# feifeibear/long-context-attention

Hardware: AMD Instinct MI355X
Metric: attention TFLOP/s (algorithmic, causal fwd+bwd) + iter ms of LongContextAttention at seqlen 64K, ulysses x ring (higher is better)
Workload: dtype bf16

## Files before the change

long-context-attention_amd/csrc/usp_flash_bwd64.hip:

```cpp
#ifdef USP_B64_TIMING
#define USP_TIMING
#endif
#include "usp_bwd_params.hpp"
#include "usp_host.hpp"
#include "usp_mfma64.hpp"

namespace usp {

#ifndef USP_B64_STATW
#define USP_B64_STATW 0
#endif
constexpr int kB64_STATW = USP_B64_STATW;
#ifndef USP_B64_DMA_PH
#define USP_B64_DMA_PH 0
#endif
constexpr int kB64_DMA_PH = USP_B64_DMA_PH;
#ifndef USP_B64_E0
#define USP_B64_E0 20
#endif
constexpr int kB64_E0 = USP_B64_E0;
#ifndef USP_B64_E1
#define USP_B64_E1 54
#endif
constexpr int kB64_E1 = USP_B64_E1;


template <int DT, bool CAUSAL>
__global__ __launch_bounds__(256, 1) void flash_bwd_dkdv64_kernel(const BwdParams ) {
  using E = Elem<DT>;
  using M = M64<DT>;
  constexpr int D = 128, OWN = 128;
  constexpr int ROWB = D * 2;
  constexpr int TILEB = kTile * ROWB;
  constexpr int STATB = 2 * kTile * 4;
  constexpr int BUFB = 2 * TILEB + STATB;
  constexpr int NBUF = 3;
  constexpr int PSLOT = 8192;
  constexpr int POFF = NBUF * BUFB;
  constexpr int NKT = D / 16, NDJ = D / 32;

  extern __shared__ __attribute__((aligned(16))) char smem_raw[];
  USP_LDS char* smem = lds_block_at_zero(smem_raw);

  const int tid = threadIdx.x;
  const int lane = tid & 63;
  const int wave = __builtin_amdgcn_readfirstlane(tid >> 6);
  const int role = wave >> 1;
  const int slice = wave & 1;
  const int l31 = lane & 31;
  const int hi = lane >> 5;
  typedef const __attribute__((address_space(4))) BwdParams* KArgs;
  KArgs p = (KArgs)__builtin_amdgcn_kernarg_segment_ptr();
  asm volatile("" : "+s"(p));

  const int dma_row = lane >> 4;
  const int dma_c8 = ((lane & 15) ^ ((lane >> 4) << 2)) * 16;
  const int q_voff = dma_row * (int)p->q_ss * 2 + dma_c8, do_voff = dma_row * (int)p->do_ss * 2 + dma_c8;
  const int rd_base = l31 * ROWB + ((hi ^ tile_swz<D>(l31)) * 16);
  int tr_addr[NDJ][2];
  {
    const int i = lane & 15, grp = (lane >> 4) & 1;
#pragma unroll
    for (int dj = 0; dj < NDJ; ++dj)
#pragma unroll
      for (int e = 0; e < 2; ++e) tr_addr[dj][e] = tr_read_offset<D>(i, grp, hi, dj, e);
  }
  USP_LDS char* pex = smem + POFF + slice * 2 * PSLOT + lane * 16;

  const ItemWalk walk(p->n_items);
  for (int pass = 0;; ++pass) {
  int w = walk.at(pass);
  if (w < 0) break;
  asm volatile("" : "+s"(p));
  USP_TM(const uint64_t tm_item = __builtin_amdgcn_s_memtime();)
  w = walk.dealt(w, p->nblk);
  const int blk = w % p->nblk;
  int rest = w / p->nblk;
  int g = 0, cut = 0;
  if (p->qsplit > 1) { cut = rest % p->qsplit; rest /= p->qsplit; }
  if (p->ngrp > 1) { g = rest % p->ngrp; rest /= p->ngrp; }
  const int hkv = rest % p->Hkv, b = rest / p->Hkv;
  const int gsub = p->gsub;
  const int h0 = hkv * p->G + g * gsub;
  const int own0 = blk * OWN;
  const int off = p->causal_off;
  const int ow = own0 + slice * 64;

  u32x4 rf[2][NKT];
  {
    const char* pr[2];
#pragma unroll
    for (int kb = 0; kb < 2; ++kb) {
      const int orow = ow + 32 * kb + l31;
      const int orow_c = orow < p->Sk ? orow : p->Sk - 1;
      pr[kb] = (role == 0 ? p->k + 2 * (b * p->k_sb + (int64_t)orow_c * p->k_ss + hkv * p->k_sh)
                          : p->v + 2 * (b * p->v_sb + (int64_t)orow_c * p->v_ss + hkv * p->v_sh)) + 16 * hi;
    }
    load_resident16(rf[0], rf[1], pr[0], pr[1]);
  }

  {
#pragma unroll
    for (int kb = 0; kb < 2; ++kb)
#pragma unroll
      for (int t = 0; t < NKT; ++t) pin_agpr4(rf[kb][t]);
  }
  const float c2 = p->scale_log2;
  const float neg_inv_scale = -__builtin_amdgcn_rcpf(p->scale);

  int t_end = (p->Sq + kTile - 1) / kTile;
  int t_begin = usp_first_row_tile(own0, CAUSAL, off, t_end, kTile);
  if (p->qsplit > 1) {
    const int per = (t_end - t_begin + p->qsplit - 1) / p->qsplit;
    t_begin = usp_run_begin(t_begin, t_end, per, cut);
    t_end = usp_run_end(t_begin, t_end, per);
  }
  const int n_iter = t_end - t_begin;

  const int64_t tb1 = (int64_t)kTile * p->q_ss * 2, tb2 = (int64_t)kTile * p->do_ss * 2;
  int q_step = 4 * (int)p->q_ss * 2 - 1024, do_step = 4 * (int)p->do_ss * 2 - 1024;
  const int q_rowb = (int)p->q_ss * 2, do_rowb = (int)p->do_ss * 2;
  const int gq = role == 0 ? slice : 2 + slice, gd = 2 * slice;
  int lds_q = gq * 4096, lds_d = TILEB + gd * 4096;
  const char *q_cur = nullptr, *do_cur = nullptr;
  int rows_q = 0, rows_d = 0;

  const float *lse_h = nullptr, *dl_h = nullptr;
  int st_row = 0;
  float st_lse = 0.f, st_delta = 0.f;
  bool st_in = false;
  const bool stat_wave = wave == kB64_STATW;
  auto pf_head = [&](int h) {
    q_cur = p->q + 2 * (b * p->q_sb + h * p->q_sh) + t_begin * tb1 + (int64_t)gq * 16 * q_rowb;
    do_cur = p->dout + 2 * (b * p->do_sb + h * p->do_sh) + t_begin * tb2 + (int64_t)gd * 16 * do_rowb;
    rows_q = p->Sq - t_begin * kTile - 16 * gq;
    rows_d = p->Sq - t_begin * kTile - 16 * gd;
    lse_h = p->lse + b * p->lse_sb + h * p->lse_sh;
    dl_h = p->delta + b * p->dl_sb + h * p->dl_sh;
    st_row = t_begin * kTile;
  };
  u32x4 q_rs, do_rs;
  int dma_buf = 0;
  auto dma_open = [&](int buf) {
    q_rs = make_rsrc_rows(q_cur, rows_q, 16, q_rowb, 2 * D);
    do_rs = make_rsrc_rows(do_cur, rows_d, 32, do_rowb, 2 * D);
    dma_buf = buf;
    q_cur += tb1;
    do_cur += tb2;
    rows_q -= kTile;
    rows_d -= kTile;
  };
  auto stats_fetch = [&]() {
    if (stat_wave) {
      const int r = st_row + lane;
      st_in = r < p->Sq;
      const int rc = st_in ? r : p->Sq - 1;
      const float* pl = lse_h + rc;
      const float* pd = dl_h + rc;
      asm volatile("global_load_dword %0, %2, off\n\tglobal_load_dword %1, %3, off" : "=&v"(st_lse), "=&v"(st_delta) : "v"(pl), "v"(pd) : "memory");
    }
    st_row += kTile;
  };
  auto dma_piece = [&](int n) {
    asm volatile("" : "+s"(lds_q), "+s"(lds_d), "+s"(q_step), "+s"(do_step));
    const int i = n & 3;
    if (n < 4) lds_dma16_asm(q_rs, lds_q + dma_buf * BUFB, q_voff ^ (16 * i), i * q_step, i);
    else if (n < 8) lds_dma16_asm(do_rs, lds_d + dma_buf * BUFB, do_voff ^ (16 * i), i * do_step, i);
    else lds_dma16_asm(do_rs, lds_d + 4096 + dma_buf * BUFB, do_voff ^ (16 * i), 4096 + 4 * do_step + i * do_step, i);
  };
  auto stats_store = [&](int buf) {
    if (stat_wave) {
      asm volatile("" : "+v"(st_lse), "+v"(st_delta));
      const float l2 = (st_in && st_lse != USP_NEG_INF) ? st_lse * neg_inv_scale : -__builtin_inff();
      *(USP_LDS float*)(smem + buf * BUFB + 2 * TILEB + 4 * lane) = l2;
      *(USP_LDS float*)(smem + buf * BUFB + 2 * TILEB + 4 * kTile + 4 * lane) = st_in ? -st_delta : 0.f;
    }
  };

  f32x16 acc[2][NDJ];
#pragma unroll
  for (int kb = 0; kb < 2; ++kb)
#pragma unroll
    for (int dj = 0; dj < NDJ; ++dj) zero_pin_agpr(acc[kb][dj]);

  const int n_mask = usp_masked_row_tiles(ow, CAUSAL, off, t_begin, n_iter, kTile);
  int tile_cur = t_begin, buf_a = 0, buf_b = NBUF - 1;
USP_TM(
  uint64_t tm_body = 0, tm_drain = 0, tm_bar = 0, tm_last = __builtin_amdgcn_s_memtime();
  const uint64_t tm_loop = tm_last;
)
  u32x4 fc0[NKT];
  f32x16 cst0;
#pragma unroll
  for (int kt = 0; kt < NKT; ++kt) fc0[kt] = u32x4{0u, 0u, 0u, 0u};
#pragma unroll
  for (int r = 0; r < 16; ++r) cst0[r] = 0.f;
  auto step = [&](auto role_c, auto mask_c, int it, bool work) __attribute__((always_inline)) {
    constexpr int ROLE = decltype(role_c)::value;
    constexpr bool MASK = decltype(mask_c)::value;
    constexpr int E0 = kB64_E0, E1 = kB64_E1;
    static_assert(E0 >= 16 && E1 <= 56 && E1 > E0, "");
    const int buf_n = buf_a + 1 == NBUF ? 0 : buf_a + 1;
    stats_fetch();
    int krn = rd_base + buf_a * BUFB + TILEB;
    asm volatile("" : "+v"(krn));
    auto next_c = [&](int kt) { fc0[kt] = *(USP_LDS const u32x4*)(smem + (krn ^ (32 * kt))); };
    auto next_s = [&](int j) {
      const f32x4 t = *(USP_LDS const f32x4*)(smem + buf_a * BUFB + 2 * TILEB + 4 * kTile + 16 * hi + 32 * j);
#pragma unroll
      for (int e = 0; e < 4; ++e) cst0[4 * j + e] = t[e];
    };
    if (work) {
#pragma unroll
      for (int kb = 0; kb < 2; ++kb)
#pragma unroll
        for (int t = 0; t < NKT; ++t) pin_agpr4(rf[kb][t]);
      const int my_it = it - ROLE;
      const int buf = ROLE == 0 ? buf_a : buf_b;
      const int s0 = (ROLE == 0 ? tile_cur : tile_cur - 1) * kTile;
      USP_LDS const char* x1 = smem + buf * BUFB;
      USP_LDS const char* x2 = x1 + TILEB;
      USP_LDS const char* xg = ROLE == 0 ? x2 : x1;
      USP_LDS const char* stat = x1 + 2 * TILEB + (ROLE == 0 ? 0 : 4 * kTile) + 16 * hi;
      USP_LDS char* pslot = pex + (my_it & 1) * PSLOT;
      f32x16 sc[2][2];
      u32x4 pk[2][2][2];
      u32x4 pin[2][2][2];
      f32x16 cst[2];
      int kr = rd_base + buf * BUFB + (ROLE == 0 ? 0 : TILEB);
      asm volatile("" : "+v"(kr));
      auto load_stats = [&](int h) {
        if (ROLE == 1 && h == 0) { cst[0] = cst0; return; }
#pragma unroll
        for (int j = 0; j < 4; ++j) {
          const f32x4 t = *(USP_LDS const f32x4*)(stat + 128 * h + 32 * j);
#pragma unroll
          for (int e = 0; e < 4; ++e) cst[h][4 * j + e] = t[e];
        }
      };
      auto elem = [&](int h, int n) {
        const int k2 = n >> 4, kb = (n >> 3) & 1, r = 8 * k2 + (n & 7);
        float val;
        if (ROLE == 0) {
          val = fast_exp2(sc[h][kb][r] * c2);
        } else {
          const uint32_t wd = pin[h][kb][k2][(r & 7) >> 1];
          val = ((r & 1) ? E::hi(wd) : E::lo(wd)) * sc[h][kb][r];
        }
        sc[h][kb][r] = val;
      };
      auto elem_pack = [&](int h, int n) {
        const int k2 = n >> 4, kb = (n >> 3) & 1, r = 8 * k2 + (n & 7);
        if (r & 1) pk[h][kb][k2][(r & 7) >> 1] = E::pack2(sc[h][kb][r - 1], sc[h][kb][r]);
        if (ROLE == 0 && (r & 7) == 7)
          *(USP_LDS u32x4*)(pslot + ((2 * h + kb) * 2 + k2) * 1024) = pk[h][kb][k2];
      };
      constexpr int LAG = ROLE == 0 ? 2 : 0;
      auto elem_slot = [&](int sl) {
        if (sl < E0 || sl >= E1) return;
#pragma unroll
        for (int n = (sl - E0) * 64 / (E1 - E0); n < (sl - E0 + 1) * 64 / (E1 - E0); ++n) {
          elem(n >> 5, n & 31);
          if (n >= LAG) elem_pack((n - LAG) >> 5, (n - LAG) & 31);
        }
        if (sl == E1 - 1) {
#pragma unroll
          for (int n = 64 - LAG; n < 64; ++n) elem_pack(n >> 5, n & 31);
        }
      };
      auto apply_mask = [&](int h) {
#pragma unroll
        for (int kb = 0; kb < 2; ++kb) {
          const int d = ow + 32 * kb + l31 - off - s0 - 4 * hi - 32 * h;
#pragma unroll
          for (int r = 0; r < 16; ++r)
            if (d > (r & 3) + 8 * (r >> 2)) sc[h][kb][r] = USP_NEG_INF;
        }
      };
      u32x4 fc[2][NKT];
      u32x4 xa[2][2 * NDJ];
      auto rd_c = [&](int h, int kt) { fc[h][kt] = *(USP_LDS const u32x4*)(smem + h * 32 * ROWB + (kr ^ (32 * kt))); };
      auto rd_g = [&](int h, int f) {
        USP_LDS const char* xb = xg + (2 * h + f / NDJ) * 16 * ROWB;
        const u32x2 a0 = lds_read_tr16(xb + tr_addr[f % NDJ][0]);
        const u32x2 a1 = lds_read_tr16(xb + tr_addr[f % NDJ][1]);
        xa[h][f] = u32x4{a0[0], a0[1], a1[0], a1[1]};
      };
      auto chain_init = [&](int h) {
        load_stats(h);
        if (ROLE == 1) {
#pragma unroll
          for (int kb = 0; kb < 2; ++kb)
#pragma unroll
            for (int k2 = 0; k2 < 2; ++k2) pin[h][kb][k2] = *(USP_LDS const u32x4*)(pslot + ((2 * h + kb) * 2 + k2) * 1024);
        }
      };
      auto chain_phase = [&](int h) {
#pragma unroll
        for (int sl = 0; sl < 16; ++sl) {
          const int kt = sl >> 1, kb = sl & 1;
          if (kt == 0) M::template s_first_c<MASK>(sc[h][kb], fc[h][kt], rf[kb][kt], cst[h]);
          else M::template s_next<MASK>(sc[h][kb], fc[h][kt], rf[kb][kt]);
          if (h == kB64_DMA_PH && sl == 0) {
            __builtin_amdgcn_sched_barrier(0);
            dma_open(buf_n);
          }
          if (sl < NKT) { if (h == 0) rd_c(1, sl); else rd_g(0, sl); }
          if (h == 0 && sl == 8) chain_init(1);
          elem_slot(16 * h + sl);
          if (h == kB64_DMA_PH) {
            if (ROLE == 0 && (sl & 3) == 1) dma_piece(sl >> 2);
            if (ROLE == 1 && sl >= 1 && sl <= 12) dma_piece(sl - 1);
          }
          __builtin_amdgcn_sched_barrier(0);
        }
      };
      auto grad_phase = [&](int h) {
#pragma unroll
        for (int i = 0; i < 16; ++i) {
          const int f = i >> 1, kb = i & 1;
          M::template o_acc<MASK>(acc[kb][f % NDJ], xa[h][f], pk[h][kb][f / NDJ]);
          if (h == 0 && i < 2 * NDJ) rd_g(1, i);
          if (ROLE == 1 && h == 1 && i >= 8) next_c(i - 8);
          if (ROLE == 1 && h == 1 && i >= 4 && i < 8) next_s(i - 4);
          elem_slot(32 + 16 * h + i);
          __builtin_amdgcn_sched_barrier(0);
        }
      };
      chain_init(0);
      if (ROLE == 1) {
#pragma unroll
        for (int kt = 0; kt < NKT; ++kt) fc[0][kt] = fc0[kt];
      } else {
#pragma unroll
        for (int kt = 0; kt < NKT; ++kt) rd_c(0, kt);
      }
      __builtin_amdgcn_sched_barrier(0);
      chain_phase(0);
      if (MASK) { mfma_settle(sc[0]); apply_mask(0); }
      __builtin_amdgcn_s_waitcnt(0xc07f);
      chain_phase(1);
      if (MASK) { mfma_settle(sc[1]); apply_mask(1); }
      __builtin_amdgcn_s_waitcnt(0xc07f);
      grad_phase(0);
      __builtin_amdgcn_s_waitcnt(0xc07f);
      grad_phase(1);
    } else {
      dma_open(buf_n);
#pragma unroll
      for (int n = 0; n < (ROLE == 0 ? 4 : 12); ++n) dma_piece(n);
    }
    if (ROLE == 1 && !work) {
#pragma unroll
      for (int kt = 0; kt < NKT; ++kt) next_c(kt);
#pragma unroll
      for (int j = 0; j < 4; ++j) next_s(j);
    }
    buf_b = buf_a;
    buf_a = buf_n;
    if (ROLE == 0 || it > 0) ++tile_cur;
    USP_TM(const uint64_t tm0 = __builtin_amdgcn_s_memtime();)
    dma_drain();
    USP_TM(const uint64_t tm1 = __builtin_amdgcn_s_memtime();)
    stats_store(buf_n);
    __syncthreads();
    USP_TM(const uint64_t tm2 = __builtin_amdgcn_s_memtime();
           tm_body += tm0 - tm_last; tm_drain += tm1 - tm0; tm_bar += tm2 - tm1; tm_last = tm2;)
  };
  const std::integral_constant<int, 0> rA;
  const std::integral_constant<int, 1> rB;
  const std::integral_constant<bool, false> plain;
  const std::integral_constant<bool, true> masked;
  auto open_head = [&](int h) {
    pf_head(h);
    stats_fetch();
    dma_open(0);
#pragma unroll
    for (int n = 0; n < 4; ++n) dma_piece(n);
    if (role == 1) {
#pragma unroll
      for (int n = 4; n < 12; ++n) dma_piece(n);
    }
    dma_drain();
    stats_store(0);
    __syncthreads();
    tile_cur = t_begin; buf_a = 0; buf_b = NBUF - 1;
  };
  if (role == 0) {
    for (int hh = 0; hh < gsub; ++hh) {
      open_head(h0 + hh);
      int it = 0;
      __builtin_amdgcn_s_waitcnt(0x0f70);
      for (; it < n_mask; ++it) step(rA, masked, it, true);
      __builtin_amdgcn_s_waitcnt(0x0f70);
      for (; it < n_iter; ++it) step(rA, plain, it, true);
      mfma_settle(acc);
      step(rA, plain, n_iter, false);
    }
  } else {
    for (int hh = 0; hh < gsub; ++hh) {
      open_head(h0 + hh);
      step(rB, plain, 0, false);
      __builtin_amdgcn_s_waitcnt(0x0f70);
      for (int it = 1; it <= n_iter; ++it) step(rB, plain, it, true);
      mfma_settle(acc);
    }
  }

  mfma_settle(acc);
USP_TM(
  const uint64_t tm_epi = __builtin_amdgcn_s_memtime();
  if (pass == 0 && lane == 0 && (blockIdx.x % 61) == 0)
    printf("TM wg %3d wave %d blk %2d n_iter %3d : body %8llu drain %7llu barrier %7llu  (per iteration %5llu / %4llu / %4llu)\n",
           (int)blockIdx.x, wave, blk, n_iter, (unsigned long long)tm_body, (unsigned long long)tm_drain,
           (unsigned long long)tm_bar, (unsigned long long)(tm_body / (n_iter + 1)), (unsigned long long)(tm_drain / (n_iter + 1)),
           (unsigned long long)(tm_bar / (n_iter + 1)));
)
  asm volatile("" : "+s"(p));
  const bool wide = !p->split && (p->wide16 & (role == 0 ? 4 : 2)) != 0;
#pragma unroll
  for (int kb = 0; kb < 2; ++kb) {
    const int orow = ow + 32 * kb + l31;
    if (wide) {
      const int orow_c = orow < p->Sk ? orow : 0;
      char* row16 = role == 0 ? p->dv16 + 2 * (b * p->dv16_sb + (int64_t)orow_c * p->dv16_ss + hkv * p->dv16_sh)
                              : p->dk16 + 2 * (b * p->dk16_sb + (int64_t)orow_c * p->dk16_ss + hkv * p->dk16_sh);
      store_row16_wide<E, NDJ>(row16, acc[kb], role == 0 ? 1.f : p->scale, hi, orow < p->Sk);
    } else if (orow < p->Sk) {
      float* o32;
      char* o16 = nullptr;
      int accf;
      const float mul = role == 0 ? 1.f : p->scale;
      if (p->split) {
        const int64_t wo = (((int64_t)(g * p->qsplit + cut) * p->ws_rows + (int64_t)b * p->Sk + orow) * p->Hkv + hkv) * D;
        o32 = (role == 0 ? p->ws_dv : p->ws_dk) + wo; accf = 0;
      } else if (role == 0) {
        o32 = p->dv + b * p->dv_sb + (int64_t)orow * p->dv_ss + hkv * p->dv_sh; accf = p->accum_dv;
        if (p->dv16) o16 = p->dv16 + 2 * (b * p->dv16_sb + (int64_t)orow * p->dv16_ss + hkv * p->dv16_sh);
      } else {
        o32 = p->dk + b * p->dk_sb + (int64_t)orow * p->dk_ss + hkv * p->dk_sh; accf = p->accum_dk;
        if (p->dk16) o16 = p->dk16 + 2 * (b * p->dk16_sb + (int64_t)orow * p->dk16_ss + hkv * p->dk16_sh);
      }
      store_row32_acc<E, NDJ>(o32, o16, acc[kb], mul, hi, accf);
    }
  }
USP_TM(
  if (pass < 3 && lane == 0 && (blockIdx.x % 61) == 0)
    printf("TI wg %3d pass %d wave %d blk %2d n_iter %3d n_mask %d : prologue %6llu loops %8llu epilogue %6llu\n", (int)blockIdx.x, pass,
           wave, blk, n_iter, n_mask, (unsigned long long)(tm_loop - tm_item), (unsigned long long)(tm_epi - tm_loop),
           (unsigned long long)(__builtin_amdgcn_s_memtime() - tm_epi));
)
  }
}

bool dkdv64_serves(const BwdParams& p_in) {
  if (p_in.seq_q || p_in.seq_k || p_in.sched || p_in.win_on) return false;
  return dma_rows_ok(p_in.q_ss, true) && dma_rows_ok(p_in.do_ss, true);
}

bool launch_dkdv64(const BwdParams& p_in, int dtype, bool causal, hipStream_t st, int* rc) {
  if (!dkdv64_serves(p_in)) return false;
  BwdParams p = p_in;
  p.wide16 = ((p.dk16 && !p.accum_dk && tensor_aligned(p.dk16, p.dk16_sb, p.dk16_ss, p.dk16_sh, 16, 8)) ? 2 : 0) |
             ((p.dv16 && !p.accum_dv && tensor_aligned(p.dv16, p.dv16_sb, p.dv16_ss, p.dv16_sh, 16, 8)) ? 4 : 0);
  p.nblk = (p.Sk + 127) / 128;
  p.n_items = p.B * p.Hkv * p.nblk * p.ngrp * p.qsplit;
  const int grid = persistent_grid(p.n_items, device_cus(), p.interleave);
  constexpr size_t lds = 3 * (2 * kTile * 128 * 2 + 2 * kTile * 4) + 2 * 2 * 8192;
  with_dtype_causal(dtype, causal, [&](auto dt, auto c) {
    hipLaunchKernelGGL((flash_bwd_dkdv64_kernel<decltype(dt)::value, decltype(c)::value>), dim3(grid), dim3(256), lds, st, p);
  });
  *rc = launched();
  return true;
}

}
```

Baseline: 1008.

## Rebalance Q/dO tile staging across waves with configurable per-wave DMA deal

Adds a compile-time table that assigns which wave stages which 16-row Q and dO groups, and at which schedule slots its DMA pieces issue. The default deal moves all staging off the role-0 waves onto the role-1 waves, each loading two Q and two dO groups. It also spreads the DMA issues across the chain and grad phases at a configurable stride instead of packing them into the chain phase. The goal is to take load-issue work off the waves on the critical path and smooth the DMA traffic through the iteration. The cost is more instantiated code paths and heavier DMA duty on the role-1 waves.

```diff
diff --git a/long-context-attention_amd/csrc/usp_flash_bwd64.hip b/long-context-attention_amd/csrc/usp_flash_bwd64.hip
--- a/long-context-attention_amd/csrc/usp_flash_bwd64.hip
+++ b/long-context-attention_amd/csrc/usp_flash_bwd64.hip
@@ -23,6 +23,52 @@
 #define USP_B64_E1 54
 #endif
 constexpr int kB64_E1 = USP_B64_E1;
+
+struct B64WaveDeal { int q0, nq, d0, nd, s0, ds; };
+struct B64Deal { B64WaveDeal w[4]; };
+constexpr B64Deal kB64_DEALS[] = {
+    {{{0, 1, 0, 0, 1, 4}, {1, 1, 0, 0, 1, 4}, {2, 1, 0, 2, 1, 1}, {3, 1, 2, 2, 1, 1}}},
+    {{{0, 0, 0, 0, 1, 4}, {0, 0, 0, 0, 1, 4}, {0, 2, 0, 2, 1, 1}, {2, 2, 2, 2, 1, 1}}},
+    {{{0, 0, 0, 0, 1, 4}, {0, 1, 0, 0, 1, 4}, {1, 2, 0, 2, 1, 1}, {3, 1, 2, 2, 1, 1}}},
+    {{{0, 0, 0, 0, 1, 4}, {0, 1, 0, 0, 1, 4}, {1, 1, 0, 2, 1, 1}, {2, 2, 2, 2, 1, 1}}},
+};
+#ifndef USP_B64_DEAL
+#define USP_B64_DEAL 1
+#endif
+#ifndef USP_B64_SPREAD
+#define USP_B64_SPREAD 3
+#endif
+#ifndef USP_B64_S0B
+#define USP_B64_S0B 1
+#endif
+constexpr B64Deal b64_deal_spread(B64Deal d, int s0, int ds) {
+  for (int w = 2; w < 4; ++w) { d.w[w].s0 = s0; d.w[w].ds = ds; }
+  return d;
+}
+constexpr B64Deal kB64_DEAL = b64_deal_spread(kB64_DEALS[USP_B64_DEAL], USP_B64_S0B, USP_B64_SPREAD);
+constexpr int b64_pieces(const B64WaveDeal& w) { return 4 * (w.nq + w.nd); }
+constexpr bool b64_deal_ok(const B64Deal& d) {
+  for (int g = 0; g < 4; ++g) {
+    int nq = 0, nd = 0;
+    for (int w = 0; w < 4; ++w) {
+      nq += (g >= d.w[w].q0 && g < d.w[w].q0 + d.w[w].nq) ? 1 : 0;
+      nd += (g >= d.w[w].d0 && g < d.w[w].d0 + d.w[w].nd) ? 1 : 0;
+    }
+    if (nq != 1 || nd != 1) return false;
+  }
+  for (int w = 0; w < 4; ++w) {
+    if (d.w[w].nq < 0 || d.w[w].nd < 0 || d.w[w].q0 < 0 || d.w[w].d0 < 0) return false;
+    if (d.w[w].q0 + d.w[w].nq > 4 || d.w[w].d0 + d.w[w].nd > 4) return false;
+    if (d.w[w].s0 < 1 || d.w[w].ds < 1) return false;
+    if (b64_pieces(d.w[w]) > 0 && 16 * kB64_DMA_PH + d.w[w].s0 + (b64_pieces(d.w[w]) - 1) * d.w[w].ds > 63) return false;
+  }
+  return true;
+}
+static_assert(b64_deal_ok(kB64_DEAL), "staging deal: every group of Q and of dO is staged by exactly one wave, every piece has a slot");
+constexpr bool b64_same_shape(const B64WaveDeal& a, const B64WaveDeal& b) {
+  return a.nq == b.nq && a.nd == b.nd && a.s0 == b.s0 && a.ds == b.ds;
+}
+constexpr bool kB64_PER_WAVE = !(b64_same_shape(kB64_DEAL.w[0], kB64_DEAL.w[1]) && b64_same_shape(kB64_DEAL.w[2], kB64_DEAL.w[3]));
 
 
 template <int DT, bool CAUSAL>
@@ -120,7 +166,9 @@
   const int64_t tb1 = (int64_t)kTile * p->q_ss * 2, tb2 = (int64_t)kTile * p->do_ss * 2;
   int q_step = 4 * (int)p->q_ss * 2 - 1024, do_step = 4 * (int)p->do_ss * 2 - 1024;
   const int q_rowb = (int)p->q_ss * 2, do_rowb = (int)p->do_ss * 2;
-  const int gq = role == 0 ? slice : 2 + slice, gd = 2 * slice;
+  constexpr B64Deal DL = kB64_DEAL;
+  const int gq = role == 0 ? DL.w[0].q0 + slice * (DL.w[1].q0 - DL.w[0].q0) : DL.w[2].q0 + slice * (DL.w[3].q0 - DL.w[2].q0);
+  const int gd = role == 0 ? DL.w[0].d0 + slice * (DL.w[1].d0 - DL.w[0].d0) : DL.w[2].d0 + slice * (DL.w[3].d0 - DL.w[2].d0);
   int lds_q = gq * 4096, lds_d = TILEB + gd * 4096;
   const char *q_cur = nullptr, *do_cur = nullptr;
   int rows_q = 0, rows_d = 0;
@@ -129,28 +177,34 @@
   int st_row = 0;
   float st_lse = 0.f, st_delta = 0.f;
   bool st_in = false;
-  const bool stat_wave = wave == kB64_STATW;
-  auto pf_head = [&](int h) {
-    q_cur = p->q + 2 * (b * p->q_sb + h * p->q_sh) + t_begin * tb1 + (int64_t)gq * 16 * q_rowb;
-    do_cur = p->dout + 2 * (b * p->do_sb + h * p->do_sh) + t_begin * tb2 + (int64_t)gd * 16 * do_rowb;
-    rows_q = p->Sq - t_begin * kTile - 16 * gq;
-    rows_d = p->Sq - t_begin * kTile - 16 * gd;
+  const bool stat_wave_rt = wave == kB64_STATW;
+  auto pf_head = [&](auto wv_c, int h) {
+    constexpr B64WaveDeal WD = kB64_DEAL.w[decltype(wv_c)::value];
+    if (WD.nq > 0) {
+      q_cur = p->q + 2 * (b * p->q_sb + h * p->q_sh) + t_begin * tb1 + (int64_t)gq * 16 * q_rowb;
+      rows_q = p->Sq - t_begin * kTile - 16 * gq;
+    }
+    if (WD.nd > 0) {
+      do_cur = p->dout + 2 * (b * p->do_sb + h * p->do_sh) + t_begin * tb2 + (int64_t)gd * 16 * do_rowb;
+      rows_d = p->Sq - t_begin * kTile - 16 * gd;
+    }
     lse_h = p->lse + b * p->lse_sb + h * p->lse_sh;
     dl_h = p->delta + b * p->dl_sb + h * p->dl_sh;
     st_row = t_begin * kTile;
   };
   u32x4 q_rs, do_rs;
   int dma_buf = 0;
-  auto dma_open = [&](int buf) {
-    q_rs = make_rsrc_rows(q_cur, rows_q, 16, q_rowb, 2 * D);
-    do_rs = make_rsrc_rows(do_cur, rows_d, 32, do_rowb, 2 * D);
+  auto dma_open = [&](auto wv_c, int buf) {
+    constexpr B64WaveDeal WD = kB64_DEAL.w[decltype(wv_c)::value];
+    if (WD.nq > 0) q_rs = make_rsrc_rows(q_cur, rows_q, 16 * WD.nq, q_rowb, 2 * D);
+    if (WD.nd > 0) do_rs = make_rsrc_rows(do_cur, rows_d, 16 * WD.nd, do_rowb, 2 * D);
     dma_buf = buf;
-    q_cur += tb1;
-    do_cur += tb2;
-    rows_q -= kTile;
-    rows_d -= kTile;
-  };
-  auto stats_fetch = [&]() {
+    if (WD.nq > 0) q_cur += tb1;
+    if (WD.nd > 0) do_cur += tb2;
+    if (WD.nq > 0) rows_q -= kTile;
+    if (WD.nd > 0) rows_d -= kTile;
+  };
+  auto stats_fetch = [&](bool stat_wave) {
     if (stat_wave) {
       const int r = st_row + lane;
       st_in = r < p->Sq;
@@ -161,14 +215,14 @@
     }
     st_row += kTile;
   };
-  auto dma_piece = [&](int n) {
+  auto dma_piece = [&](auto wv_c, int n) {
+    constexpr B64WaveDeal WD = kB64_DEAL.w[decltype(wv_c)::value];
     asm volatile("" : "+s"(lds_q), "+s"(lds_d), "+s"(q_step), "+s"(do_step));
-    const int i = n & 3;
-    if (n < 4) lds_dma16_asm(q_rs, lds_q + dma_buf * BUFB, q_voff ^ (16 * i), i * q_step, i);
-    else if (n < 8) lds_dma16_asm(do_rs, lds_d + dma_buf * BUFB, do_voff ^ (16 * i), i * do_step, i);
-    else lds_dma16_asm(do_rs, lds_d + 4096 + dma_buf * BUFB, do_voff ^ (16 * i), 4096 + 4 * do_step + i * do_step, i);
-  };
-  auto stats_store = [&](int buf) {
+    const int i = n & 3, j = n >> 2, jd = j - WD.nq;
+    if (j < WD.nq) lds_dma16_asm(q_rs, lds_q + 4096 * j + dma_buf * BUFB, q_voff ^ (16 * i), j * (4096 + 4 * q_step) + i * q_step, i);
+    else lds_dma16_asm(do_rs, lds_d + 4096 * jd + dma_buf * BUFB, do_voff ^ (16 * i), jd * (4096 + 4 * do_step) + i * do_step, i);
+  };
+  auto stats_store = [&](bool stat_wave, int buf) {
     if (stat_wave) {
       asm volatile("" : "+v"(st_lse), "+v"(st_delta));
       const float l2 = (st_in && st_lse != USP_NEG_INF) ? st_lse * neg_inv_scale : -__builtin_inff();
@@ -195,13 +249,21 @@
   for (int kt = 0; kt < NKT; ++kt) fc0[kt] = u32x4{0u, 0u, 0u, 0u};
 #pragma unroll
   for (int r = 0; r < 16; ++r) cst0[r] = 0.f;
-  auto step = [&](auto role_c, auto mask_c, int it, bool work) __attribute__((always_inline)) {
-    constexpr int ROLE = decltype(role_c)::value;
+  auto step = [&](auto wv_c, auto mask_c, int it, bool work) __attribute__((always_inline)) {
+    constexpr int WV = decltype(wv_c)::value;
+    constexpr int ROLE = WV >> 1;
     constexpr bool MASK = decltype(mask_c)::value;
+    constexpr B64WaveDeal WD = kB64_DEAL.w[WV];
+    constexpr int NP = b64_pieces(WD);
+    const bool stat_wave = kB64_PER_WAVE ? WV == kB64_STATW : stat_wave_rt;
     constexpr int E0 = kB64_E0, E1 = kB64_E1;
     static_assert(E0 >= 16 && E1 <= 56 && E1 > E0, "");
     const int buf_n = buf_a + 1 == NBUF ? 0 : buf_a + 1;
-    stats_fetch();
+    stats_fetch(stat_wave);
+    auto dma_slot = [&](int sl) {
+      const int r = sl - 16 * kB64_DMA_PH - WD.s0;
+      if (r >= 0 && r % WD.ds == 0 && r / WD.ds < NP) dma_piece(wv_c, r / WD.ds);
+    };
     int krn = rd_base + buf_a * BUFB + TILEB;
     asm volatile("" : "+v"(krn));
     auto next_c = [&](int kt) { fc0[kt] = *(USP_LDS const u32x4*)(smem + (krn ^ (32 * kt))); };
@@ -303,15 +365,12 @@
           else M::template s_next<MASK>(sc[h][kb], fc[h][kt], rf[kb][kt]);
           if (h == kB64_DMA_PH && sl == 0) {
             __builtin_amdgcn_sched_barrier(0);
-            dma_open(buf_n);
+            dma_open(wv_c, buf_n);
           }
           if (sl < NKT) { if (h == 0) rd_c(1, sl); else rd_g(0, sl); }
           if (h == 0 && sl == 8) chain_init(1);
           elem_slot(16 * h + sl);
-          if (h == kB64_DMA_PH) {
-            if (ROLE == 0 && (sl & 3) == 1) dma_piece(sl >> 2);
-            if (ROLE == 1 && sl >= 1 && sl <= 12) dma_piece(sl - 1);
-          }
+          dma_slot(16 * h + sl);
           __builtin_amdgcn_sched_barrier(0);
         }
       };
@@ -324,6 +383,7 @@
           if (ROLE == 1 && h == 1 && i >= 8) next_c(i - 8);
           if (ROLE == 1 && h == 1 && i >= 4 && i < 8) next_s(i - 4);
           elem_slot(32 + 16 * h + i);
+          dma_slot(32 + 16 * h + i);
           __builtin_amdgcn_sched_barrier(0);
         }
       };
@@ -346,9 +406,9 @@
       __builtin_amdgcn_s_waitcnt(0xc07f);
       grad_phase(1);
     } else {
-      dma_open(buf_n);
-#pragma unroll
-      for (int n = 0; n < (ROLE == 0 ? 4 : 12); ++n) dma_piece(n);
+      dma_open(wv_c, buf_n);
+#pragma unroll
+      for (int n = 0; n < NP; ++n) dma_piece(wv_c, n);
     }
     if (ROLE == 1 && !work) {
 #pragma unroll
@@ -362,49 +422,59 @@
     USP_TM(const uint64_t tm0 = __builtin_amdgcn_s_memtime();)
     dma_drain();
     USP_TM(const uint64_t tm1 = __builtin_amdgcn_s_memtime();)
-    stats_store(buf_n);
+    stats_store(stat_wave, buf_n);
     __syncthreads();
     USP_TM(const uint64_t tm2 = __builtin_amdgcn_s_memtime();
            tm_body += tm0 - tm_last; tm_drain += tm1 - tm0; tm_bar += tm2 - tm1; tm_last = tm2;)
   };
-  const std::integral_constant<int, 0> rA;
-  const std::integral_constant<int, 1> rB;
+  const std::integral_constant<int, 0> w0;
+  const std::integral_constant<int, 1> w1;
+  const std::integral_constant<int, 2> w2;
+  const std::integral_constant<int, 3> w3;
   const std::integral_constant<bool, false> plain;
   const std::integral_constant<bool, true> masked;
-  auto open_head = [&](int h) {
-    pf_head(h);
-    stats_fetch();
-    dma_open(0);
-#pragma unroll
-    for (int n = 0; n < 4; ++n) dma_piece(n);
-    if (role == 1) {
-#pragma unroll
-      for (int n = 4; n < 12; ++n) dma_piece(n);
-    }
+  auto open_head = [&](auto wv_c, int h) __attribute__((always_inline)) {
+    constexpr int WV = decltype(wv_c)::value;
+    const bool stat_wave = kB64_PER_WAVE ? WV == kB64_STATW : stat_wave_rt;
+    pf_head(wv_c, h);
+    stats_fetch(stat_wave);
+    dma_open(wv_c, 0);
+#pragma unroll
+    for (int n = 0; n < b64_pieces(kB64_DEAL.w[WV]); ++n) dma_piece(wv_c, n);
     dma_drain();
-    stats_store(0);
+    stats_store(stat_wave, 0);
     __syncthreads();
     tile_cur = t_begin; buf_a = 0; buf_b = NBUF - 1;
   };
-  if (role == 0) {
+  auto stream_a = [&](auto wv_c) __attribute__((always_inline)) {
     for (int hh = 0; hh < gsub; ++hh) {
-      open_head(h0 + hh);
+      open_head(wv_c, h0 + hh);
       int it = 0;
       __builtin_amdgcn_s_waitcnt(0x0f70);
-      for (; it < n_mask; ++it) step(rA, masked, it, true);
+      for (; it < n_mask; ++it) step(wv_c, masked, it, true);
       __builtin_amdgcn_s_waitcnt(0x0f70);
-      for (; it < n_iter; ++it) step(rA, plain, it, true);
+      for (; it < n_iter; ++it) step(wv_c, plain, it, true);
       mfma_settle(acc);
-      step(rA, plain, n_iter, false);
-    }
+      step(wv_c, plain, n_iter, false);
+    }
+  };
+  auto stream_b = [&](auto wv_c) __attribute__((always_inline)) {
+    for (int hh = 0; hh < gsub; ++hh) {
+      open_head(wv_c, h0 + hh);
+      step(wv_c, plain, 0, false);
+      __builtin_amdgcn_s_waitcnt(0x0f70);
+      for (int it = 1; it <= n_iter; ++it) step(wv_c, plain, it, true);
+      mfma_settle(acc);
+    }
+  };
+  if (!kB64_PER_WAVE) {
+    if (role == 0) stream_a(w0);
+    else stream_b(w2);
   } else {
-    for (int hh = 0; hh < gsub; ++hh) {
-      open_head(h0 + hh);
-      step(rB, plain, 0, false);
-      __builtin_amdgcn_s_waitcnt(0x0f70);
-      for (int it = 1; it <= n_iter; ++it) step(rB, plain, it, true);
-      mfma_settle(acc);
-    }
+    if (wave == 0) stream_a(w0);
+    else if (wave == 1) stream_a(w1);
+    else if (wave == 2) stream_b(w2);
+    else stream_b(w3);
   }
 
   mfma_settle(acc);
```

Result: no change. 1010, median of 6 (+0.1%).
